# YuhuaXu/ImageMosaicing

Measured on AMD Instinct MI355X. Metric: image-pairs/sec (detect+match+H+warp), 4000x3000 UAV frames, higher is better.
Workload: dtype i16 fixed-point pyramid filtered in f32 (as the reference's OpenCV), f32 (RANSAC / warp coordinates), int8 MFMA with int32 accumulation (descriptor distances, exact), u8 (pixels); 1 GPU; C3: ONE 500-frame 4000x3000 UAV survey, pair window 2 (499 pairs), SIFT(2000,3,0.01,20) + exact BF match + 3x3 grid select + Ransac2D + MosaicImagesRefined warp; frames=500, pairs=499, frames_per_gpu=500, pairs_per_gpu=499

## Files before the change

imagemosaicing_amd/csrc/sift.hip:

```cpp
#include "common.h"
#include "sift_plan.h"
#include <memory>
#include "detmath.h"
#include <cmath>
#include <type_traits>

namespace {

using namespace sift_plan;
constexpr int MAX_INTERP = 5, ORI_BINS = 36;
constexpr int FIXPT_SCALE = 48;
constexpr float DOG_THRESHOLD_P1 = 21.0f;
constexpr float HIST_Q = 1024.0f;
constexpr int SIFT_BATCH_MAX = MI355_SIFT_BATCH_MAX;
static_assert(SIFT_BATCH_MAX == BATCH_MAX, "sift_plan.h: BATCH_MAX");
typedef int16_t lvl_t;

__host__ __device__ __forceinline__ int reflect101(int p, int n) {
    if (n == 1) return 0;
    while (p < 0 || p >= n) { if (p < 0) p = -p; else p = 2 * n - 2 - p; }
    return p;
}

typedef float v2f __attribute__((ext_vector_type(2)));
// ... 89 lines not shown
        for (int j = 1; j <= R; j++) {
            const v4f sm = *reinterpret_cast<const v4f*>(mid + j * PMID) + *reinterpret_cast<const v4f*>(mid - j * PMID);
            const v4f p = sm * a.k[R + j];
            acc = acc + p;
        }
        const int gx = x0 + 4 * xg, gy = y0 + yy;
        if (gy >= a.h) continue;
        const int o0 = sat16(acc.x), o1 = sat16(acc.y), o2 = sat16(acc.z), o3 = sat16(acc.w);
        lvl_t* d = dst + (size_t)gy * a.w + gx;
        if (gx + 3 < a.w && (a.w & 3) == 0) {
            *reinterpret_cast<uint2*>(d) = make_uint2((unsigned)(o0 & 0xffff) | ((unsigned)o1 << 16), (unsigned)(o2 & 0xffff) | ((unsigned)o3 << 16));
        } else {
            if (gx < a.w) d[0] = (lvl_t)o0;
            if (gx + 1 < a.w) d[1] = (lvl_t)o1;
            if (gx + 2 < a.w) d[2] = (lvl_t)o2;
            if (gx + 3 < a.w) d[3] = (lvl_t)o3;
        }
        if (a.ds && !(gy & 1) && (gy >> 1) < (a.h >> 1)) {
            lvl_t* q = a.ds + (size_t)fr * a.fstride + (size_t)(gy >> 1) * (a.w >> 1);
            if ((gx >> 1) < (a.w >> 1)) q[gx >> 1] = (lvl_t)o0;
            if (((gx + 2) >> 1) < (a.w >> 1)) q[(gx + 2) >> 1] = (lvl_t)o2;
        }
    }
}

#include "build/blur16_asm.inc"
template <int R, bool BGR, bool DS>
__device__ __forceinline__ void blur16_stream_body(const Blur16Args& a, int L, int nstrip, int nseg) {
    constexpr int RA = (R + 3) / 4 * 4, SW = 256, BW = SW + 2 * RA;
    constexpr int BUF = (BW + 8 + 63) & ~63;
    static_assert(2 * RA + R <= 64, "halo lanes");
    __shared__ __attribute__((aligned(16))) float s_buf[4][2][BUF];
    const int lane = threadIdx.x & 63, wave = threadIdx.x >> 6;
    int unit = __builtin_amdgcn_readfirstlane(xcd_remap(blockIdx.x, gridDim.x) * 4 + wave);
    const int per = nstrip * nseg, fr = unit / per;
    if (fr >= a.nb) return;
    unit -= fr * per;
    const int seg = unit / nstrip, strip = unit - seg * nstrip;
    if (seg >= nseg) return;
    const int x0 = strip * SW, y0 = seg * L;
    const int lact = (a.h - y0 < L) ? a.h - y0 : L;
    const int wv = a.w - x0;
    const int xm = x0 + 4 * lane;
    const int xl = xm < a.w - 4 ? xm : a.w - 4;
    int hcol, hpos;
    if (lane < RA) { hcol = x0 - RA + lane; hpos = lane; }
    else if (lane < 2 * RA) { hcol = x0 + SW + (lane - RA); hpos = SW + lane; }
    else if (wv < SW && lane < 2 * RA + R) { hcol = x0 + wv + (lane - 2 * RA); hpos = RA + wv + (lane - 2 * RA); }
    else { hcol = x0; hpos = BW + (lane & 7); }
    hcol = reflect101(hcol, a.w);
    const size_t fro = (size_t)fr * a.fstride;
    const uint8_t* bgr = a.bgr[0]; int bws = a.bgr_ws[0];
    if (BGR) {
#pragma unroll
        for (int q = 1; q < SIFT_BATCH_MAX; q++) if (fr == q) { bgr = a.bgr[q]; bws = a.bgr_ws[q]; }
    }
    const int rowb = BGR ? bws : 2 * a.w;
    int gy = y0 - R, dir = 1;
    if (gy < 0) { gy = -gy; dir = -1; }
    const unsigned long long rp = (unsigned long long)(BGR ? reinterpret_cast<uintptr_t>(bgr) : reinterpret_cast<uintptr_t>(a.src + fro)) + (unsigned long long)gy * (unsigned)rowb;
    const unsigned moff = BGR ? 3u * xl : 2u * xl;
    unsigned hoff, hsh = 0;
    if (BGR) {
        const int b0 = 3 * hcol; int st = b0 & ~3; if (st + 8 > bws) st = bws - 8;
        hoff = (unsigned)st; hsh = 8u * (unsigned)(b0 - st);
    } else hoff = 2u * hcol;
    const unsigned lds0 = (unsigned)reinterpret_cast<uintptr_t>(&s_buf[wave][0][0]);
    const unsigned lds_win = lds0 + 16u * lane, lds_main = lds0 + 4u * (RA + 4 * lane), lds_halo = lds0 + 4u * hpos;
    const unsigned long long dp = (unsigned long long)reinterpret_cast<uintptr_t>(a.dst + fro) + 2ull * (unsigned long long)y0 * a.w;
    const unsigned long long dsp = DS ? (unsigned long long)reinterpret_cast<uintptr_t>(a.ds + fro) + 2ull * (unsigned long long)(y0 >> 1) * (a.w >> 1) : 0ull;
    const unsigned doff = 2u * xm, dsoff = 2u * (xm >> 1);
    const unsigned long long smask = __ballot(xm < a.w);
    const unsigned long long kp = (unsigned long long)reinterpret_cast<uintptr_t>(__builtin_amdgcn_kernarg_segment_ptr()) + offsetof(Blur16Args, kp);
    const int n = lact + 2 * R + 1;
    const int hm1 = a.h - 1, dstr = 2 * a.w;
    (void)hsh;
#define BLUR_ASM_CALL(NAME) NAME(lds_win, lds_main, lds_halo, moff, hoff, doff, dsoff, rp, dp, dsp, kp, smask, rowb, gy, dir, hm1, dstr, n)
    if constexpr (BGR) { static_assert(R == 6, "base level"); blur16_asm_r6_bgr(lds_win, lds_main, lds_halo, moff, hoff, doff, dsoff, hsh, rp, dp, dsp, kp, smask, rowb, gy, dir, hm1, dstr, n); }
    else if constexpr (R == 5) BLUR_ASM_CALL(blur16_asm_r5);
    else if constexpr (R == 6) BLUR_ASM_CALL(blur16_asm_r6);
    else if constexpr (R == 8 && DS) BLUR_ASM_CALL(blur16_asm_r8_ds);
    else if constexpr (R == 8) BLUR_ASM_CALL(blur16_asm_r8);
    else if constexpr (R == 10) BLUR_ASM_CALL(blur16_asm_r10);
    else if constexpr (R == 13) BLUR_ASM_CALL(blur16_asm_r13);
#undef BLUR_ASM_CALL
}
template <int R, bool BGR, bool DS, int W>
__global__ __launch_bounds__(256) __attribute__((amdgpu_waves_per_eu(W, W))) void blur16_stream(Blur16Args a, int L, int nstrip, int nseg) {
    blur16_stream_body<R, BGR, DS>(a, L, nstrip, nseg);
}

__global__ __launch_bounds__(256) void downsample16(const lvl_t* src, int sw, lvl_t* dst, int dw, int dh, size_t fstride) {
    src += (size_t)blockIdx.z * fstride; dst += (size_t)blockIdx.z * fstride;
    const int x = blockIdx.x * 64 + (threadIdx.x & 63), y = blockIdx.y * 4 + (threadIdx.x >> 6);
    if (x < dw && y < dh) dst[(size_t)y * dw + x] = src[(size_t)(2 * y) * sw + 2 * x];
}

struct OctaveDev { lvl_t* lv[N_LEVELS]; int w, h; };

constexpr int ECAP = 128;
constexpr int REG_STRIDE = 32;
struct BatchStride { size_t pyr, claimed, cand, refined, kps, cube, sel, mins; };
struct FrameOuts { mi355_keypoint* kp[SIFT_BATCH_MAX]; uint8_t* d8[SIFT_BATCH_MAX]; };

struct Refined { int o, layer, r, c; float xi, xr, xc, contr, scl; unsigned start; };

struct PyrDev { OctaveDev oc[MAX_OCT]; unsigned* claimed[MAX_OCT]; unsigned* mins[MAX_OCT]; int n_oct; };

__device__ __forceinline__ float dogv(const OctaveDev& oc, size_t foff, int lvl, int r, int c) {
    const size_t o = foff + (size_t)r * oc.w + c;
    return (float)((int)oc.lv[lvl + 1][o] - (int)oc.lv[lvl][o]);
}

__device__ __forceinline__ void solve3(const float a[3][3], const float b[3], float x[3]) {
    const float det = (a[0][0] * (a[1][1] * a[2][2] - a[2][1] * a[1][2]) - a[0][1] * (a[1][0] * a[2][2] - a[2][0] * a[1][2])) + a[0][2] * (a[1][0] * a[2][1] - a[2][0] * a[1][1]);
    if (det == 0.0f) { x[0] = x[1] = x[2] = 0.0f; return; }
    const float d = 1.0f / det;
    x[0] = d * ((b[0] * (a[1][1] * a[2][2] - a[1][2] * a[2][1]) - a[0][1] * (b[1] * a[2][2] - a[1][2] * b[2])) + a[0][2] * (b[1] * a[2][1] - a[1][1] * b[2]));
    x[1] = d * ((a[0][0] * (b[1] * a[2][2] - a[1][2] * b[2]) - b[0] * (a[1][0] * a[2][2] - a[1][2] * a[2][0])) + a[0][2] * (a[1][0] * b[2] - b[1] * a[2][0]));
    x[2] = d * ((a[0][0] * (a[1][1] * b[2] - b[1] * a[2][1]) - a[0][1] * (a[1][0] * b[2] - b[1] * a[2][0])) + b[0] * (a[1][0] * a[2][1] - a[1][1] * a[2][0]));
}

struct FitOff { float xi, xr, xc; };
template <class DV>
__device__ __forceinline__ FitOff fit_step(DV dv, int L, int R, int C) {
    const float img_scale = 1.0f / (float)(255 * FIXPT_SCALE);
    const float deriv_scale = img_scale * 0.5f, second_scale = img_scale, cross_scale = img_scale * 0.25f;
    float dD[3];
    dD[0] = (dv(L, R, C + 1) - dv(L, R, C - 1)) * deriv_scale;
    dD[1] = (dv(L, R + 1, C) - dv(L, R - 1, C)) * deriv_scale;
    dD[2] = (dv(L + 1, R, C) - dv(L - 1, R, C)) * deriv_scale;
    const float v2 = dv(L, R, C) * 2.0f;
    const float dxx = (dv(L, R, C + 1) + dv(L, R, C - 1) - v2) * second_scale;
    const float dyy = (dv(L, R + 1, C) + dv(L, R - 1, C) - v2) * second_scale;
    const float dss = (dv(L + 1, R, C) + dv(L - 1, R, C) - v2) * second_scale;
    const float dxy = (dv(L, R + 1, C + 1) - dv(L, R + 1, C - 1) - dv(L, R - 1, C + 1) + dv(L, R - 1, C - 1)) * cross_scale;
    const float dxs = (dv(L + 1, R, C + 1) - dv(L + 1, R, C - 1) - dv(L - 1, R, C + 1) + dv(L - 1, R, C - 1)) * cross_scale;
    const float dys = (dv(L + 1, R + 1, C) - dv(L + 1, R - 1, C) - dv(L - 1, R + 1, C) + dv(L - 1, R - 1, C)) * cross_scale;
    const float A[3][3] = {{dxx, dxy, dxs}, {dxy, dyy, dys}, {dxs, dys, dss}};
    float X[3];
    solve3(A, dD, X);
    FitOff f; f.xi = -X[2]; f.xr = -X[1]; f.xc = -X[0];
    return f;
}
template <class DV>
__device__ __forceinline__ bool fit_accept(DV dv, int L, int R, int C, FitOff f, float contrast_thr, float edge_thr, float& contr) {
    const float img_scale = 1.0f / (float)(255 * FIXPT_SCALE);
    const float deriv_scale = img_scale * 0.5f, second_scale = img_scale, cross_scale = img_scale * 0.25f;
    float dD0 = (dv(L, R, C + 1) - dv(L, R, C - 1)) * deriv_scale;
    float dD1 = (dv(L, R + 1, C) - dv(L, R - 1, C)) * deriv_scale;
    float dD2 = (dv(L + 1, R, C) - dv(L - 1, R, C)) * deriv_scale;
    const float t = ((0.0f + dD0 * f.xc) + dD1 * f.xr) + dD2 * f.xi;
    contr = dv(L, R, C) * img_scale + t * 0.5f;
    if (fabsf(contr) * (float)N_LAYERS < contrast_thr) return false;
    const float v2 = dv(L, R, C) * 2.0f;
    const float dxx = (dv(L, R, C + 1) + dv(L, R, C - 1) - v2) * second_scale;
    const float dyy = (dv(L, R + 1, C) + dv(L, R - 1, C) - v2) * second_scale;
    const float dxy = (dv(L, R + 1, C + 1) - dv(L, R + 1, C - 1) - dv(L, R - 1, C + 1) + dv(L, R - 1, C - 1)) * cross_scale;
    const float tr = dxx + dyy, det = dxx * dyy - dxy * dxy;
    if (det <= 0.0f || (tr * tr) * edge_thr >= ((edge_thr + 1.0f) * (edge_thr + 1.0f)) * det) return false;
    return true;
}
__device__ __forceinline__ int fit_state(FitOff f) {
    if (fabsf(f.xi) < 0.5f && fabsf(f.xr) < 0.5f && fabsf(f.xc) < 0.5f) return 0;
    if (fabsf(f.xi) > 7.0e8f || fabsf(f.xr) > 7.0e8f || fabsf(f.xc) > 7.0e8f) return 1;
    if (!(f.xi == f.xi) || !(f.xr == f.xr) || !(f.xc == f.xc)) return 1;
    return 2;
}

__global__ __launch_bounds__(256) void extrema_kernel(OctaveDev oc, int octave, unsigned long long* cand, unsigned* count, unsigned cap, unsigned* overflow, BatchStride bs,
                                                      float* cube, unsigned cube_cap) {
    {
        const size_t f = blockIdx.y;
#pragma unroll
        for (int l = 0; l < N_LEVELS; l++) oc.lv[l] += f * bs.pyr;
        cand += f * bs.cand; count += f * CCNT_STRIDE; overflow += f * CNT_STRIDE; cube += f * bs.cube;
    }
    constexpr int PC = EW + 8;
    constexpr int P4 = PC / 4;
    constexpr int RW = EH + 2;
    __shared__ v4f s_d4[5][RW * P4];
    __shared__ unsigned long long s_list[ECAP];
    __shared__ unsigned s_n, s_base;
    const int tid = threadIdx.x;
    const int tiles_x = (oc.w + EW - 1) / EW, tiles_y = (oc.h + EH - 1) / EH;
    const int tile = xcd_remap(blockIdx.x, tiles_x * tiles_y);
    const int tyy = tile / tiles_x, txx = tile - tyy * tiles_x;
    const int x0 = txx * EW, y0 = tyy * EH;
    if (tid == 0) s_n = 0;
    const bool vec = ((oc.w & 3) == 0) && (x0 - 4 >= 0) && (x0 + EW + 4 <= oc.w) && ((reinterpret_cast<uintptr_t>(oc.lv[0]) & 7) == 0);
    if (vec) {
        for (int idx = tid; idx < RW * (EW / 4); idx += 256) {
            const int ry = idx / (EW / 4), c4 = idx - ry * (EW / 4);
            int gy = y0 - 1 + ry;
            gy = gy < 0 ? 0 : (gy > oc.h - 1 ? oc.h - 1 : gy);
            const size_t o = (size_t)gy * oc.w + (x0 + 4 * c4);
            v4f g[N_LEVELS];
#pragma unroll
            for (int l = 0; l < N_LEVELS; l++) g[l] = ld4(oc.lv[l] + o);
#pragma unroll
            for (int l = 0; l < 5; l++) s_d4[l][ry * P4 + 1 + c4] = g[l + 1] - g[l];
        }
        if (tid < 2 * RW) {
            const int ry = tid >> 1, side = tid & 1;
            int gy = y0 - 1 + ry;
            gy = gy < 0 ? 0 : (gy > oc.h - 1 ? oc.h - 1 : gy);
            const size_t o = (size_t)gy * oc.w + (side ? x0 + EW : x0 - 1);
            float g[N_LEVELS];
#pragma unroll
            for (int l = 0; l < N_LEVELS; l++) g[l] = ld1(oc.lv[l] + o);
#pragma unroll
            for (int l = 0; l < 5; l++) reinterpret_cast<float*>(s_d4[l])[ry * PC + (side ? 4 + EW : 3)] = g[l + 1] - g[l];
        }
    } else {
        for (int idx = tid; idx < RW * PC; idx += 256) {
            const int ry = idx / PC, rx = idx - ry * PC;
            int gy = y0 - 1 + ry, gx = x0 - 4 + rx;
            gy = gy < 0 ? 0 : (gy > oc.h - 1 ? oc.h - 1 : gy);
            gx = gx < 0 ? 0 : (gx > oc.w - 1 ? oc.w - 1 : gx);
            const size_t o = (size_t)gy * oc.w + gx;
            float g[N_LEVELS];
#pragma unroll
            for (int l = 0; l < N_LEVELS; l++) g[l] = ld1(oc.lv[l] + o);
#pragma unroll
            for (int l = 0; l < 5; l++) reinterpret_cast<float*>(s_d4[l])[idx] = g[l + 1] - g[l];
        }
    }
    __syncthreads();
    for (int item = tid; item < EH * (EW / 4); item += 256) {
        const int ly = item / (EW / 4), xg = item - ly * (EW / 4);
        const int r = y0 + ly;
        float cm[5][6], cn[5][6], mid[5][6], top[5][6], bot[5][6];
#pragma unroll
        for (int pl = 0; pl < 5; pl++) {
            const float* base = reinterpret_cast<const float*>(s_d4[pl]) + (ly + 1) * PC + 4 * xg + 4;
#pragma unroll
            for (int rr = -1; rr <= 1; rr++) {
                const float* q = base + rr * PC;
                const v4f c4 = *reinterpret_cast<const v4f*>(q);
                float v[6] = {q[-1], c4.x, c4.y, c4.z, c4.w, q[4]};
#pragma unroll
                for (int j = 0; j < 6; j++) { if (rr == -1) top[pl][j] = v[j]; else if (rr == 0) mid[pl][j] = v[j]; else bot[pl][j] = v[j]; }
            }
#pragma unroll
            for (int j = 0; j < 6; j++) {
                cm[pl][j] = fmaxf(fmaxf(top[pl][j], mid[pl][j]), bot[pl][j]);
                cn[pl][j] = fminf(fminf(top[pl][j], mid[pl][j]), bot[pl][j]);
            }
        }
        unsigned hit = 0;
#pragma unroll
        for (int k = 0; k < 4; k++) {
            const int j = k + 1;
#pragma unroll
            for (int layer = 1; layer <= N_LAYERS; layer++) {
                const float val = mid[layer][j];
                float mx = fmaxf(fmaxf(cm[layer - 1][j - 1], cm[layer - 1][j]), cm[layer - 1][j + 1]);
                mx = fmaxf(mx, fmaxf(fmaxf(cm[layer + 1][j - 1], cm[layer + 1][j]), cm[layer + 1][j + 1]));
                mx = fmaxf(mx, fmaxf(fmaxf(cm[layer][j - 1], cm[layer][j + 1]), fmaxf(top[layer][j], bot[layer][j])));
                float mn = fminf(fminf(cn[layer - 1][j - 1], cn[layer - 1][j]), cn[layer - 1][j + 1]);
                mn = fminf(mn, fminf(fminf(cn[layer + 1][j - 1], cn[layer + 1][j]), cn[layer + 1][j + 1]));
                mn = fminf(mn, fminf(fminf(cn[layer][j - 1], cn[layer][j + 1]), fminf(top[layer][j], bot[layer][j])));
                const float q = val > 0.0f ? mx : -mn;
                hit |= fabsf(val) >= fmaxf(q, DOG_THRESHOLD_P1) ? (1u << ((layer - 1) * 4 + k)) : 0u;
            }
        }
        unsigned cmask = 0;
#pragma unroll
        for (int k = 0; k < 4; k++) { const int c = x0 + 4 * xg + k; cmask |= (c >= IMG_BORDER && c < oc.w - IMG_BORDER) ? (0x111u << k) : 0u; }
        hit = (r >= IMG_BORDER && r < oc.h - IMG_BORDER) ? (hit & cmask) : 0u;
        while (hit) {
            const int bb = __builtin_ctz(hit); hit &= hit - 1;
            const int layer = bb / 4 + 1, c = x0 + 4 * xg + (bb & 3);
            const unsigned long long rec = ((unsigned long long)octave << 48) | ((unsigned long long)layer << 40) | ((unsigned long long)r << 20) | (unsigned long long)c;
            const unsigned slot = atomicAdd(&s_n, 1u);
            if (slot < ECAP) s_list[slot] = rec;
            else {
                const unsigned reg = ((unsigned)tile >> REG_SHIFT) & (NREG - 1);
                const unsigned g = atomicAdd(&count[reg * REG_STRIDE], 1u);
                if (g < cap) cand[(size_t)reg * cap + g] = rec; else *overflow = 1;
            }
        }
    }
    __syncthreads();
    const unsigned nloc = s_n < ECAP ? s_n : ECAP;
    const unsigned reg = ((unsigned)tile >> REG_SHIFT) & (NREG - 1);
    if (tid == 0 && nloc) s_base = atomicAdd(&count[reg * REG_STRIDE], nloc);
    __syncthreads();
    for (unsigned i = tid; i < nloc; i += 256) {
        const unsigned g = s_base + i;
        if (g < cap) cand[(size_t)reg * cap + g] = s_list[i] | (g < cube_cap ? (1ull << 63) : 0ull); else *overflow = 1;
    }
    for (unsigned idx = tid; idx < nloc * 27; idx += 256) {
        const unsigned ci = idx / 27, e = idx - ci * 27;
        const unsigned g = s_base + ci;
        if (g >= cube_cap) continue;
        const unsigned long long rec = s_list[ci];
        const int L0 = (int)((rec >> 40) & 0xff), R0 = (int)((rec >> 20) & 0xfffff), C0 = (int)(rec & 0xfffff);
        const int dl = (int)(e / 9) - 1, dr = (int)((e / 3) % 3) - 1, dc = (int)(e % 3) - 1;
        cube[((size_t)reg * 32 + e) * cube_cap + g] = reinterpret_cast<const float*>(s_d4[L0 + dl])[(R0 + dr - y0 + 1) * PC + (C0 + dc - x0) + 4];
    }
}

constexpr int XCAP = 512;
typedef short s2 __attribute__((ext_vector_type(2)));
struct XRow { uint2 m[N_LEVELS]; };
struct XDog { s2 m[5][2]; };
__device__ __forceinline__ s2 as_s2(unsigned v) { return __builtin_bit_cast(s2, v); }
__device__ __forceinline__ unsigned as_u(s2 v) { return __builtin_bit_cast(unsigned, v); }
__device__ __forceinline__ s2 pmax(s2 a, s2 b) { return __builtin_elementwise_max(a, b); }
__device__ __forceinline__ s2 pmin(s2 a, s2 b) { return __builtin_elementwise_min(a, b); }
__device__ __forceinline__ unsigned dpp_lower(unsigned v) { return (unsigned)__builtin_amdgcn_update_dpp(0, (int)v, 0x138 , 0xf, 0xf, true); }
__device__ __forceinline__ unsigned dpp_upper(unsigned v) { return (unsigned)__builtin_amdgcn_update_dpp(0, (int)v, 0x130 , 0xf, 0xf, true); }

__device__ __forceinline__ unsigned xtest_row(const XDog& A, const XDog& B, const XDog& C, int xm, int clo, int chi, bool row_ok) {
    s2 hx[5][2], hn[5][2];
#pragma unroll
    for (int p = 0; p < 5; p++) {
        auto h3 = [](s2 c01, s2 c23, bool mx, s2& o01, s2& o23) {
            const unsigned u01 = as_u(c01), u23 = as_u(c23);
            const unsigned l23 = dpp_lower(u23), r01 = dpp_upper(u01);
            const s2 s_m0 = as_s2(__builtin_amdgcn_alignbit(u01, l23, 16));
            const s2 s_12 = as_s2(__builtin_amdgcn_alignbit(u23, u01, 16));
            const s2 s_34 = as_s2(__builtin_amdgcn_alignbit(r01, u23, 16));
            if (mx) { o01 = pmax(pmax(s_m0, c01), s_12); o23 = pmax(pmax(s_12, c23), s_34); }
            else    { o01 = pmin(pmin(s_m0, c01), s_12); o23 = pmin(pmin(s_12, c23), s_34); }
        };
        h3(pmax(pmax(A.m[p][0], B.m[p][0]), C.m[p][0]), pmax(pmax(A.m[p][1], B.m[p][1]), C.m[p][1]), true, hx[p][0], hx[p][1]);
        h3(pmin(pmin(A.m[p][0], B.m[p][0]), C.m[p][0]), pmin(pmin(A.m[p][1], B.m[p][1]), C.m[p][1]), false, hn[p][0], hn[p][1]);
    }
    unsigned hit = 0;
    const s2 t21 = {21, 21}, tm21 = {-21, -21};
#pragma unroll
    for (int layer = 1; layer <= N_LAYERS; layer++) {
#pragma unroll
        for (int r = 0; r < 2; r++) {
            const s2 val = B.m[layer][r];
            const s2 mx = pmax(pmax(pmax(hx[layer - 1][r], hx[layer][r]), hx[layer + 1][r]), t21);
            const s2 mn = pmin(pmin(pmin(hn[layer - 1][r], hn[layer][r]), hn[layer + 1][r]), tm21);
            const bool h0 = (val.x == mx.x) | (val.x == mn.x), h1 = (val.y == mx.y) | (val.y == mn.y);
            hit = (hit << 2) | (h0 ? 2u : 0u) | (h1 ? 1u : 0u);
        }
    }
    if (!row_ok || hit == 0) return 0u;
    unsigned out = 0;
#pragma unroll
    for (int b = 0; b < 12; b++) out |= ((hit >> (11 - b)) & 1u) << b;
    unsigned cmask = 0;
#pragma unroll
    for (int k = 0; k < 4; k++) cmask |= (xm + k >= clo && xm + k < chi) ? (0x111u << k) : 0u;
    return out & cmask;
}

struct XH { s2 hx[5][2], hn[5][2]; };
struct XCen { s2 v[3][2]; };
__device__ __forceinline__ void xrow_extremes(const XDog& d, XH& h, XCen& c) {
#pragma unroll
    for (int p = 0; p < 5; p++) {
        const unsigned u01 = as_u(d.m[p][0]), u23 = as_u(d.m[p][1]);
        const unsigned l23 = dpp_lower(u23), r01 = dpp_upper(u01);
        const s2 s_m0 = as_s2(__builtin_amdgcn_alignbit(u01, l23, 16));
        const s2 s_12 = as_s2(__builtin_amdgcn_alignbit(u23, u01, 16));
        const s2 s_34 = as_s2(__builtin_amdgcn_alignbit(r01, u23, 16));
        h.hx[p][0] = pmax(pmax(s_m0, d.m[p][0]), s_12); h.hx[p][1] = pmax(pmax(s_12, d.m[p][1]), s_34);
        h.hn[p][0] = pmin(pmin(s_m0, d.m[p][0]), s_12); h.hn[p][1] = pmin(pmin(s_12, d.m[p][1]), s_34);
    }
#pragma unroll
    for (int l = 0; l < 3; l++) { c.v[l][0] = d.m[l + 1][0]; c.v[l][1] = d.m[l + 1][1]; }
}
__device__ __forceinline__ unsigned xtest_rows(const XH& A, const XH& B, const XH& C, const XCen& cen, int xm, int clo, int chi, bool row_ok) {
    s2 hx[5][2], hn[5][2];
#pragma unroll
    for (int p = 0; p < 5; p++)
#pragma unroll
        for (int r = 0; r < 2; r++) { hx[p][r] = pmax(pmax(A.hx[p][r], B.hx[p][r]), C.hx[p][r]); hn[p][r] = pmin(pmin(A.hn[p][r], B.hn[p][r]), C.hn[p][r]); }
    unsigned hit = 0;
    const s2 t21 = {21, 21}, tm21 = {-21, -21};
#pragma unroll
    for (int layer = 1; layer <= N_LAYERS; layer++) {
#pragma unroll
        for (int r = 0; r < 2; r++) {
            const s2 val = cen.v[layer - 1][r];
            const s2 mx = pmax(pmax(pmax(hx[layer - 1][r], hx[layer][r]), hx[layer + 1][r]), t21);
            const s2 mn = pmin(pmin(pmin(hn[layer - 1][r], hn[layer][r]), hn[layer + 1][r]), tm21);
            const bool h0 = (val.x == mx.x) | (val.x == mn.x), h1 = (val.y == mx.y) | (val.y == mn.y);
            hit = (hit << 2) | (h0 ? 2u : 0u) | (h1 ? 1u : 0u);
        }
    }
    if (!row_ok || hit == 0) return 0u;
    unsigned out = 0;
#pragma unroll
    for (int b = 0; b < 12; b++) out |= ((hit >> (11 - b)) & 1u) << b;
    unsigned cmask = 0;
#pragma unroll
    for (int k = 0; k < 4; k++) cmask |= (xm + k >= clo && xm + k < chi) ? (0x111u << k) : 0u;
    return out & cmask;
}

__global__ __launch_bounds__(256) __attribute__((amdgpu_waves_per_eu(XWAVES, XWAVES)))
void extrema_stream(OctaveDev oc, int octave, unsigned long long* cand, unsigned* count, unsigned cap, unsigned* overflow, BatchStride bs,
                    float* cube, unsigned cube_cap, int L, int nstrip, int nseg, int nb, int xsw ) {
    const int lane = threadIdx.x & 63, wave = threadIdx.x >> 6;
    int unit = __builtin_amdgcn_readfirstlane(xcd_remap(blockIdx.x, gridDim.x) * 4 + wave);
    const int per = nstrip * nseg, fr = unit / per;
    if (fr >= nb) return;
    unit -= fr * per;
    {
        const size_t f = (size_t)fr;
#pragma unroll
        for (int l = 0; l < N_LEVELS; l++) oc.lv[l] += f * bs.pyr;
        cand += f * bs.cand; count += f * CCNT_STRIDE; overflow += f * CNT_STRIDE; cube += f * bs.cube;
    }
    const int seg = unit / nstrip, strip = unit - seg * nstrip;
    const int xs = strip * xsw, y0 = seg * L;
    const int lact = (oc.h - y0 < L) ? oc.h - y0 : L;
    const unsigned reg = (unsigned)unit & (NREG - 1);
    const int xm = xs - 4 + 4 * lane;
    const int xl = xm < 0 ? 0 : (xm < oc.w - 4 ? xm : oc.w - 4);
    int clo = xs > IMG_BORDER ? xs : IMG_BORDER, chi = xs + xsw < oc.w - IMG_BORDER ? xs + xsw : oc.w - IMG_BORDER;
    if (lane == 0 || lane == 63) { clo = 0; chi = 0; }
    const int hm1 = oc.h - 1;
    auto load_row = [&](int r, XRow& q) {
        r = r < 0 ? 0 : (r > hm1 ? hm1 : r);
        const size_t o = (size_t)r * oc.w + xl;
#pragma unroll
        for (int l = 0; l < N_LEVELS; l++) q.m[l] = *reinterpret_cast<const uint2*>(oc.lv[l] + o);
    };
    auto to_dog = [&](const XRow& q, XDog& d) {
#pragma unroll
        for (int p = 0; p < 5; p++) { d.m[p][0] = as_s2(q.m[p + 1].x) - as_s2(q.m[p].x); d.m[p][1] = as_s2(q.m[p + 1].y) - as_s2(q.m[p].y); }
    };
    __shared__ unsigned long long s_rec[4][XCAP];
    int nq = 0;
    auto wave_sync = [&]() { __builtin_amdgcn_fence(__ATOMIC_ACQ_REL, "wavefront"); __builtin_amdgcn_wave_barrier(); };
    auto flush = [&]() {
        if (nq == 0) return;
        wave_sync();
        unsigned base = 0;
        if (lane == 0) base = atomicAdd(&count[reg * REG_STRIDE], (unsigned)nq);
        base = __shfl(base, 0);
        for (int idx = lane; idx < nq; idx += 64) {
            const unsigned g = base + (unsigned)idx;
            if (g >= cap) { *overflow = 1; continue; }
            cand[(size_t)reg * cap + g] = s_rec[wave][idx];
        }
        wave_sync();
        nq = 0;
    };
    auto emit = [&](unsigned hit, int rc, auto in_loop) -> bool {
        constexpr bool IN_LOOP = decltype(in_loop)::value;
        const int nq0 = nq;
        while (__builtin_amdgcn_ballot_w64(hit != 0)) {
            const bool mine = hit != 0;
            const int bb = mine ? __builtin_ctz(hit) : 0;
            hit &= hit - 1;
            const unsigned long long m = __builtin_amdgcn_ballot_w64(mine);
            const int add = __builtin_popcountll(m);
            if (nq + add > XCAP) {
                if constexpr (IN_LOOP) { nq = nq0; return false; }
                else flush();
            }
            if (mine) {
                const int layer = bb / 4 + 1, c = xm + (bb & 3);
                s_rec[wave][nq + __builtin_popcountll(m & ((1ull << lane) - 1ull))] =
                    ((unsigned long long)octave << 48) | ((unsigned long long)layer << 40) | ((unsigned long long)rc << 20) | (unsigned long long)c;
            }
            nq += add;
        }
        return true;
    };
    XH win[3];
    XCen cen[3];
    XRow nxt[XD];
    {
        XRow q; XDog dq;
        load_row(y0 - 1, q); to_dog(q, dq); xrow_extremes(dq, win[0], cen[0]);
        load_row(y0, q); to_dog(q, dq); xrow_extremes(dq, win[1], cen[1]);
#pragma unroll
        for (int d = 0; d < XD; d++) load_row(y0 + 1 + d, nxt[d]);
    }
    int tb = 0, t_slow = -1;
    for (bool done = false; !done;) {
        for (;;) {
            if (tb >= lact) { done = true; break; }
            if (nq > XCAP / 2) break;
            auto step = [&](auto jc) -> bool {
                constexpr int j = decltype(jc)::value;
                const int tt = tb + j;
                if (tt >= lact) return false;
                const int rc = y0 + tt;
                XH& A = win[j % 3]; XH& B = win[(j + 1) % 3]; XH& Cc = win[(j + 2) % 3];
                { XDog dq; to_dog(nxt[j % XD], dq); xrow_extremes(dq, Cc, cen[(j + 2) % 3]); }
                load_row(rc + 1 + XD, nxt[j % XD]);
                const unsigned hit = xtest_rows(A, B, Cc, cen[(j + 1) % 3], xm, clo, chi, rc >= IMG_BORDER && rc < oc.h - IMG_BORDER);
                if (!emit(hit, rc, std::true_type{})) { t_slow = tt; return false; }
                return true;
            };
            if (!static_rows<0, 3 * XD>(step)) { done = true; break; }
            tb += 3 * XD;
        }
        flush();
    }
    if (t_slow >= 0) {
        for (int tt = t_slow; tt < lact; tt++) {
            const int rc = y0 + tt;
            XRow q; XDog A, B, Cc;
            load_row(rc - 1, q); to_dog(q, A);
            load_row(rc, q); to_dog(q, B);
            load_row(rc + 1, q); to_dog(q, Cc);
            emit(xtest_row(A, B, Cc, xm, clo, chi, rc >= IMG_BORDER && rc < oc.h - IMG_BORDER), rc, std::false_type{});
        }
        flush();
    }
}

__global__ __launch_bounds__(256) void refine_kernel(PyrDev P, const unsigned long long* cand_all, const unsigned* cand_counts, unsigned cand_cap, unsigned* cand_total,
                                                     float contrast_thr, float edge_thr, float sigma,
                                                     Refined* out, unsigned* out_count, unsigned out_cap, unsigned* out_resp, BatchStride bs,
                                                     const float* cube_all, unsigned cube_cap) {
    const size_t fr = blockIdx.z, foff = fr * bs.pyr;
    cube_all += fr * bs.cube;
    cand_all += fr * bs.cand; cand_counts += fr * CCNT_STRIDE; cand_total += fr * CNT_STRIDE;
    out += fr * bs.refined; out_count += fr * CNT_STRIDE; out_resp += fr * bs.refined;
    const unsigned reg = blockIdx.y;
    unsigned n = cand_counts[reg * REG_STRIDE];
    if (n > cand_cap) n = cand_cap;
    const unsigned long long* cand = cand_all + (size_t)reg * cand_cap;
    if (blockIdx.x == 0 && blockIdx.y == 0 && threadIdx.x < 64) {
        unsigned tot = cand_counts[threadIdx.x * REG_STRIDE];
        for (int off = 32; off > 0; off >>= 1) tot += __shfl_xor(tot, off);
        if (threadIdx.x == 0) cand_total[0] = tot;
    }
    for (unsigned i = blockIdx.x * blockDim.x + threadIdx.x; i < n; i += gridDim.x * blockDim.x) {
        const unsigned long long pk = cand[i];
        const int o = (int)((pk >> 48) & 0xff);
        int L = (int)((pk >> 40) & 0xff), R = (int)((pk >> 20) & 0xfffff), C = (int)(pk & 0xfffff);
        const unsigned start = ((unsigned)L << 28) | ((unsigned)R << 14) | (unsigned)C;
        const OctaveDev& oc = P.oc[o];
        auto dv = [&](int l, int r, int c) { return dogv(oc, foff, l, r, c); };
        FitOff f = {0.0f, 0.0f, 0.0f};
        int it = 0;
        bool alive = true, accepted = false;
        float contr = 0.0f;
        const bool from_cube = (pk >> 63) != 0;
        const bool can_gather = (oc.w & 1) == 0 && (foff & 1) == 0;
        float cv[27];
        auto gather = [&](int l, int r, int c) {
            const int a0 = (c - 1) & ~1, sh = ((c - 1) & 1) * 16;
            int v[4][9];
#pragma unroll
            for (int q = 0; q < 4; q++) {
                const lvl_t* lp = oc.lv[l - 1 + q] + foff;
#pragma unroll
                for (int dr = 0; dr < 3; dr++) {
                    const uint2_a4 wv = *reinterpret_cast<const uint2_a4*>(lp + (size_t)(r - 1 + dr) * oc.w + a0);
                    const unsigned long long ww = (((unsigned long long)wv.y << 32) | wv.x) >> sh;
                    v[q][dr * 3 + 0] = (int)(short)(ww & 0xffffu); v[q][dr * 3 + 1] = (int)(short)((ww >> 16) & 0xffffu); v[q][dr * 3 + 2] = (int)(short)((ww >> 32) & 0xffffu);
                }
            }
#pragma unroll
            for (int dl = 0; dl < 3; dl++)
#pragma unroll
                for (int e = 0; e < 9; e++) cv[dl * 9 + e] = (float)(v[dl + 1][e] - v[dl][e]);
        };
        if (from_cube || can_gather) {
            for (; it < MAX_INTERP; it++) {
                if (it == 0 && from_cube) {
                    const float* cb = cube_all + (size_t)reg * 32 * cube_cap + i;
#pragma unroll
                    for (int e = 0; e < 27; e++) cv[e] = cb[(size_t)e * cube_cap];
                } else if (can_gather) gather(L, R, C);
                else break;
                const int L0 = L, R0 = R, C0 = C;
                auto dvc = [&](int l, int r, int c) { return cv[(l - L0 + 1) * 9 + (r - R0 + 1) * 3 + (c - C0 + 1)]; };
                f = fit_step(dvc, L, R, C);
                const int stt = fit_state(f);
                if (stt == 1) { alive = false; break; }
                if (stt == 0) { accepted = fit_accept(dvc, L, R, C, f, contrast_thr, edge_thr, contr); alive = accepted; break; }
                C += (int)rintf(f.xc); R += (int)rintf(f.xr); L += (int)rintf(f.xi);
                if (L < 1 || L > N_LAYERS || C < IMG_BORDER || C >= oc.w - IMG_BORDER || R < IMG_BORDER || R >= oc.h - IMG_BORDER) { alive = false; break; }
            }
            if (!alive || (can_gather && !accepted)) continue;
        }
        if (!accepted) {
            for (; it < MAX_INTERP; it++) {
                f = fit_step(dv, L, R, C);
                const int stt = fit_state(f);
                if (stt == 0) break;
                if (stt == 1) { alive = false; break; }
                C += (int)rintf(f.xc); R += (int)rintf(f.xr); L += (int)rintf(f.xi);
                if (L < 1 || L > N_LAYERS || C < IMG_BORDER || C >= oc.w - IMG_BORDER || R < IMG_BORDER || R >= oc.h - IMG_BORDER) { alive = false; break; }
            }
            if (!alive || it >= MAX_INTERP) continue;
            if (!fit_accept(dv, L, R, C, f, contrast_thr, edge_thr, contr)) continue;
        }
        const size_t bit = ((size_t)R * oc.w + C) * 4 + (size_t)L;
        const unsigned mask = 1u << (bit & 31);
        if (!P.mins[o]) {
            const unsigned old = atomicOr(&P.claimed[o][fr * bs.claimed + (bit >> 5)], mask);
            if (old & mask) continue;
        }
        const unsigned long long act = __ballot(1);
        const int leader = __builtin_ctzll(act), lane_id = (int)(threadIdx.x & 63);
        unsigned slot = 0;
        if (lane_id == leader) slot = atomicAdd(out_count, (unsigned)__builtin_popcountll(act));
        slot = __shfl(slot, leader) + (unsigned)__builtin_popcountll(act & ((1ull << lane_id) - 1ull));
        if (slot < out_cap) {
            Refined rr;
            rr.o = o; rr.layer = L; rr.r = R; rr.c = C; rr.xi = f.xi; rr.xr = f.xr; rr.xc = f.xc; rr.contr = contr;
            rr.scl = sigma * det_exp2f(((float)L + f.xi) / (float)N_LAYERS);
            rr.start = start;
            out[slot] = rr;
            out_resp[slot] = __float_as_uint(fabsf(contr));
            if (P.mins[o]) atomicMin(&P.mins[o][fr * bs.mins + bit], start);
        } else if (!P.mins[o]) atomicAnd(&P.claimed[o][fr * bs.claimed + (bit >> 5)], ~mask);
    }
}

__device__ __forceinline__ void unclaim_body(const PyrDev& P, const Refined* ref, const unsigned* ref_count, unsigned ref_cap, const BatchStride& bs, size_t fr, unsigned first, unsigned step) {
    ref += fr * bs.refined; ref_count += fr * CNT_STRIDE;
    unsigned n = *ref_count;
    if (n > ref_cap) n = ref_cap;
    for (unsigned i = first; i < n; i += step) {
        const Refined rr = ref[i];
        const size_t bit = ((size_t)rr.r * P.oc[rr.o].w + rr.c) * 4 + (size_t)rr.layer;
        atomicAnd(&P.claimed[rr.o][fr * bs.claimed + (bit >> 5)], ~(1u << (bit & 31)));
    }
}

__global__ __launch_bounds__(256) void keepall_live_kernel(PyrDev P, const Refined* ref, const unsigned* ref_count, unsigned ref_cap, unsigned* ctrl, unsigned* list, BatchStride bs) {
    const size_t fr = blockIdx.y;
    ref += fr * bs.refined; ref_count += fr * CNT_STRIDE; ctrl += fr * CNT_STRIDE; list += fr * bs.refined;
    unsigned n = *ref_count;
    if (n > ref_cap) n = ref_cap;
    const int lane = threadIdx.x & 63;
    for (unsigned i0 = blockIdx.x * blockDim.x; i0 < n; i0 += gridDim.x * blockDim.x) {
        const unsigned i = i0 + threadIdx.x;
        bool take = false;
        if (i < n) {
            const Refined rr = ref[i];
            const size_t bit = ((size_t)rr.r * P.oc[rr.o].w + rr.c) * 4 + (size_t)rr.layer;
            take = P.mins[rr.o][fr * bs.mins + bit] == rr.start;
        }
        const unsigned long long m = __builtin_amdgcn_ballot_w64(take);
        if (m) {
            const int first = __builtin_ctzll(m);
            unsigned base = 0;
            if (lane == first) base = atomicAdd(&ctrl[2], (unsigned)__builtin_popcountll(m));
            base = __shfl(base, first);
            if (take) list[base + (unsigned)__builtin_popcountll(m & ((1ull << lane) - 1ull))] = i;
        }
    }
}
__global__ __launch_bounds__(256) void keepall_reset_kernel(PyrDev P, const Refined* ref, const unsigned* ref_count, unsigned ref_cap, BatchStride bs) {
    const size_t fr = blockIdx.y;
    ref += fr * bs.refined; ref_count += fr * CNT_STRIDE;
    unsigned n = *ref_count;
    if (n > ref_cap) n = ref_cap;
    for (unsigned i = blockIdx.x * blockDim.x + threadIdx.x; i < n; i += gridDim.x * blockDim.x) {
        const Refined rr = ref[i];
        P.mins[rr.o][fr * bs.mins + ((size_t)rr.r * P.oc[rr.o].w + rr.c) * 4 + (size_t)rr.layer] = 0xffffffffu;
    }
}

struct KpRec {
    unsigned resp_bits; int o, layer, r, c, bin;
    float ptx, pty, scl, angle, xi;
    unsigned start;
};

constexpr int UNCLAIM_WGS = 32;
__global__ __launch_bounds__(1024) void select_unclaim_kernel(PyrDev P, const Refined* ref, BatchStride bs,
                                                              const unsigned* resp , const unsigned* ref_count, unsigned ref_cap,
                                                              unsigned want, unsigned* ctrl , size_t resp_stride,
                                                              unsigned* list ) {
    if (blockIdx.x > 0) { unclaim_body(P, ref, ref_count, ref_cap, bs, blockIdx.y, (blockIdx.x - 1) * 1024 + threadIdx.x, (gridDim.x - 1) * 1024); return; }
    resp += (size_t)blockIdx.y * resp_stride; ref_count += (size_t)blockIdx.y * CNT_STRIDE; ctrl += (size_t)blockIdx.y * CNT_STRIDE;
    list += (size_t)blockIdx.y * resp_stride;
    __shared__ unsigned s_h[16][256];
    __shared__ unsigned s_sel[2], s_cnt;
    const int tid = threadIdx.x, wv = tid >> 6;
    unsigned n = *ref_count;
    if (n > ref_cap) n = ref_cap;
    if (n <= want) {
        if (tid == 0) { ctrl[0] = 0; ctrl[1] = 0; ctrl[2] = n; }
        for (unsigned i = tid; i < n; i += 1024) list[i] = i;
        return;
    }
    const unsigned nr = (n + 1023u) & ~1023u;
    unsigned above = 0, hi_sel = 0;
    for (int pass = 0; pass < 2; pass++) {
        for (int i = tid; i < 16 * 256; i += 1024) (&s_h[0][0])[i] = 0;
        __syncthreads();
        for (unsigned i0 = tid; i0 < nr; i0 += 8 * 1024) {
            unsigned vv[8];
#pragma unroll
            for (int u = 0; u < 8; u++) { const unsigned i = i0 + 1024u * u; vv[u] = i < n ? resp[i] : 0u; }
#pragma unroll
            for (int u = 0; u < 8; u++) {
                if (i0 + 1024u * u >= n) continue;
                const unsigned key = (vv[u] >> 15) & 0xffffu;
                if (pass == 0) atomicAdd(&s_h[wv][key >> 8], 1u);
                else if ((key >> 8) == hi_sel) atomicAdd(&s_h[wv][key & 255u], 1u);
            }
        }
        __syncthreads();
        if (tid < 256) { unsigned t = 0; for (int w = 0; w < 16; w++) t += s_h[w][tid]; s_h[0][tid] = t; }
        __syncthreads();
        if (tid == 0) {
            unsigned cum = above; int b = 255;
            for (; b >= 0; b--) { if (cum + s_h[0][b] >= want) break; cum += s_h[0][b]; }
            if (b < 0) b = 0;
            s_sel[0] = (unsigned)b; s_sel[1] = cum;
        }
        __syncthreads();
        if (pass == 0) { hi_sel = s_sel[0]; above = s_sel[1]; }
        else if (tid == 0) { ctrl[0] = ((hi_sel << 8) | s_sel[0]) << 15; ctrl[1] = 0; s_cnt = 0; }
        __syncthreads();
    }
    const unsigned T = ((hi_sel << 8) | s_sel[0]) << 15;
    const int lane = tid & 63;
    for (unsigned i0 = tid; i0 < nr; i0 += 8 * 1024) {
        unsigned vv[8];
#pragma unroll
        for (int u = 0; u < 8; u++) { const unsigned i = i0 + 1024u * u; vv[u] = i < n ? resp[i] : 0u; }
#pragma unroll
        for (int u = 0; u < 8; u++) {
            const unsigned i = i0 + 1024u * u;
            const bool take = i < n && vv[u] >= T;
            const unsigned long long m = __builtin_amdgcn_ballot_w64(take);
            if (m) {
                const int first = __builtin_ctzll(m);
                unsigned base = 0;
                if (lane == first) base = atomicAdd(&s_cnt, (unsigned)__builtin_popcountll(m));
                base = __shfl(base, first);
                if (take) list[base + (unsigned)__builtin_popcountll(m & ((1ull << lane) - 1ull))] = i;
            }
        }
    }
    __syncthreads();
    if (tid == 0) ctrl[2] = s_cnt;
}

constexpr int OCAP = 256;
__global__ __launch_bounds__(256) void orient_kernel(PyrDev P, const Refined* ref, const unsigned* ref_count, unsigned ref_cap,
                                                     KpRec* out, unsigned* out_resp, unsigned* out_count, unsigned out_cap,
                                                     const unsigned* ctrl, int pass, BatchStride bs, const unsigned* list) {
    const size_t fr = blockIdx.y, foff = fr * bs.pyr;
    ref += fr * bs.refined; ref_count += fr * CNT_STRIDE; out += fr * bs.kps; out_resp += fr * bs.kps; out_count += fr * CNT_STRIDE; ctrl += fr * CNT_STRIDE;
    list += fr * bs.refined;
    __shared__ unsigned long long s_hq[4][ORI_BINS];
    const unsigned Tbits = ctrl[0];
    if (pass == 1 && (ctrl[1] == 0 || Tbits == 0)) return;
    __shared__ float s_hist[4][ORI_BINS + 4];
    __shared__ KpRec s_out[OCAP];
    __shared__ unsigned s_on, s_obase;
    const int tid = threadIdx.x, lane = tid & 63, wv = tid >> 6;
    unsigned n = *ref_count;
    if (n > ref_cap) n = ref_cap;
    if (pass == 0) n = ctrl[2] < n ? ctrl[2] : n;
    if (tid == 0) s_on = 0;
    __syncthreads();
    for (unsigned base = blockIdx.x * 4; base < n; base += gridDim.x * 4) {
        unsigned k = base + wv;
        bool take = false;
        if (k < n) {
            if (pass == 0) { k = list[k]; take = true; }
            else take = __float_as_uint(fabsf(ref[k].contr)) < Tbits;
        }
        if (take) {
            const Refined rr = ref[k];
            const OctaveDev& oc = P.oc[rr.o];
            const lvl_t* img = oc.lv[rr.layer] + foff;
            const int radius = (int)rintf(4.5f * rr.scl);
            const float osig = 1.5f * rr.scl;
            const float expf_scale = -1.0f / (2.0f * osig * osig);
            const int side = 2 * radius + 1, S = side * side;
            if (lane < ORI_BINS) s_hq[wv][lane] = 0ull;
            __builtin_amdgcn_fence(__ATOMIC_ACQ_REL, "workgroup");
            __builtin_amdgcn_wave_barrier();
            const int per = (S + 63) / 64;
            int sc = lane * per, ic = sc / side, jc = sc - ic * side;
            for (int k0 = 0; k0 < per; k0 += 4) {
                float dxv[4], dyv[4]; int d2v[4]; bool okv[4];
#pragma unroll
                for (int u = 0; u < 4; u++) {
                    const int s = k0 + u < per ? sc : S;
                    const int i = ic - radius, j = jc - radius;
                    sc++; jc++;
                    if (jc == side) { jc = 0; ic++; }
                    const int y = rr.r + i, x = rr.c + j;
                    okv[u] = (s < S) && !(y <= 0 || y >= oc.h - 1 || x <= 0 || x >= oc.w - 1);
                    d2v[u] = i * i + j * j;
                    dxv[u] = 0.0f; dyv[u] = 0.0f;
                    if (okv[u]) {
                        dxv[u] = (float)((int)img[(size_t)y * oc.w + x + 1] - (int)img[(size_t)y * oc.w + x - 1]);
                        dyv[u] = (float)((int)img[(size_t)(y - 1) * oc.w + x] - (int)img[(size_t)(y + 1) * oc.w + x]);
                    }
                }
#pragma unroll
                for (int u = 0; u < 4; u++) {
                    if (!okv[u]) continue;
                    const float dx = dxv[u], dy = dyv[u];
                    const float wgt = det_expf((float)d2v[u] * expf_scale);
                    const float ang = det_atan2deg(dy, dx);
                    const float mag = sqrtf(dx * dx + dy * dy);
                    int b = (int)rintf(((float)ORI_BINS / 360.0f) * ang);
                    if (b >= ORI_BINS) b -= ORI_BINS;
                    if (b < 0) b += ORI_BINS;
                    const float t = wgt * mag;
                    atomicAdd(&s_hq[wv][b], (unsigned long long)(long long)(int)rintf(t * HIST_Q));
                }
            }
            __builtin_amdgcn_fence(__ATOMIC_ACQ_REL, "workgroup");
            __builtin_amdgcn_wave_barrier();
// ... 779 lines not shown
```

Before: 3899 image-pairs/s.

## Capture 3x3x3 DoG neighbourhood cubes in extrema stream via LDS ring

The streaming extrema kernel now keeps the last three DoG rows in a per-wave LDS ring buffer. When a candidate is emitted, it copies the 27-value neighbourhood into LDS, and the flush writes those values into the cube array, setting the cube-valid bit on each candidate. This lets refinement reuse the cubes instead of re-reading the pyramid. It also shrinks XCAP and the flush threshold so LDS stays within budget. The cost is extra LDS writes on every row, added wave syncs in emit, more frequent flushes, and cubes only for the first 64 candidates per flush.

```diff
diff --git a/imagemosaicing_amd/csrc/sift.hip b/imagemosaicing_amd/csrc/sift.hip
--- a/imagemosaicing_amd/csrc/sift.hip
+++ b/imagemosaicing_amd/csrc/sift.hip
@@ -415,7 +415,12 @@
     }
 }
 
-constexpr int XCAP = 512;
+constexpr int XCAP = 144;
+constexpr int XNB_CAP = 64;
+constexpr int XRING_DW = 5 * 3 * 128;
+constexpr int XNB_DW = 18;
+constexpr int XLDS_BYTES = 4 * (XRING_DW * 4 + XCAP * 8 + XNB_CAP * XNB_DW * 4);
+static_assert(XWAVES * XLDS_BYTES <= 160 * 1024 && XLDS_BYTES <= 53 * 1024, "extrema_stream: ring + list must leave room for XWAVES workgroups per CU");
 typedef short s2 __attribute__((ext_vector_type(2)));
 struct XRow { uint2 m[N_LEVELS]; };
 struct XDog { s2 m[5][2]; };
@@ -543,10 +548,19 @@
 #pragma unroll
         for (int p = 0; p < 5; p++) { d.m[p][0] = as_s2(q.m[p + 1].x) - as_s2(q.m[p].x); d.m[p][1] = as_s2(q.m[p + 1].y) - as_s2(q.m[p].y); }
     };
+    __shared__ unsigned s_ring[4][XRING_DW];
     __shared__ unsigned long long s_rec[4][XCAP];
+    __shared__ uint2 s_nb[4][XNB_CAP][XNB_DW / 2];
+    static_assert(sizeof(s_ring) + sizeof(s_rec) + sizeof(s_nb) == XLDS_BYTES, "XLDS_BYTES");
+    auto ring_put = [&](const XDog& d, int slot) {
+        unsigned* q = &s_ring[wave][lane * 30 + slot];
+#pragma unroll
+        for (int p = 0; p < 5; p++) { q[p * 3] = as_u(d.m[p][0]); q[p * 3 + 15] = as_u(d.m[p][1]); }
+    };
     int nq = 0;
     auto wave_sync = [&]() { __builtin_amdgcn_fence(__ATOMIC_ACQ_REL, "wavefront"); __builtin_amdgcn_wave_barrier(); };
-    auto flush = [&]() {
+    auto flush = [&](auto cubes) {
+        constexpr bool CUBES = decltype(cubes)::value;
         if (nq == 0) return;
         wave_sync();
         unsigned base = 0;
@@ -555,13 +569,28 @@
         for (int idx = lane; idx < nq; idx += 64) {
             const unsigned g = base + (unsigned)idx;
             if (g >= cap) { *overflow = 1; continue; }
-            cand[(size_t)reg * cap + g] = s_rec[wave][idx];
+            const unsigned long long rec = s_rec[wave][idx];
+            const bool has = CUBES && idx < XNB_CAP && g < cube_cap;
+            cand[(size_t)reg * cap + g] = rec | (has ? (1ull << 63) : 0ull);
+            if (has) {
+                const int sh = (rec & 1ull) ? 0 : 16;
+                float* cb = cube + (size_t)reg * 32 * cube_cap + g;
+#pragma nounroll
+                for (int i = 0; i < XNB_DW / 2; i++, cb += (size_t)3 * cube_cap) {
+                    const uint2 wv = s_nb[wave][idx][i];
+                    const unsigned long long ww = (((unsigned long long)wv.y << 32) | wv.x) >> sh;
+                    cb[0] = (float)(int)(short)(ww & 0xffffu);
+                    cb[cube_cap] = (float)(int)(short)((ww >> 16) & 0xffffu);
+                    cb[(size_t)2 * cube_cap] = (float)(int)(short)((ww >> 32) & 0xffffu);
+                }
+            }
         }
         wave_sync();
         nq = 0;
     };
-    auto emit = [&](unsigned hit, int rc, auto in_loop) -> bool {
-        constexpr bool IN_LOOP = decltype(in_loop)::value;
+    auto emit = [&](unsigned hit, int rc, auto sbc) -> bool {
+        constexpr int SB = decltype(sbc)::value;
+        constexpr bool IN_LOOP = SB >= 0;
         const int nq0 = nq;
         while (__builtin_amdgcn_ballot_w64(hit != 0)) {
             const bool mine = hit != 0;
@@ -571,12 +600,27 @@
             const int add = __builtin_popcountll(m);
             if (nq + add > XCAP) {
                 if constexpr (IN_LOOP) { nq = nq0; return false; }
-                else flush();
-            }
+                else flush(std::false_type{});
+            }
+            if constexpr (IN_LOOP) wave_sync();
             if (mine) {
-                const int layer = bb / 4 + 1, c = xm + (bb & 3);
-                s_rec[wave][nq + __builtin_popcountll(m & ((1ull << lane) - 1ull))] =
-                    ((unsigned long long)octave << 48) | ((unsigned long long)layer << 40) | ((unsigned long long)rc << 20) | (unsigned long long)c;
+                const int layer = bb / 4 + 1, k = bb & 3, c = xm + k;
+                const int slot = nq + __builtin_popcountll(m & ((1ull << lane) - 1ull));
+                s_rec[wave][slot] = ((unsigned long long)octave << 48) | ((unsigned long long)layer << 40) | ((unsigned long long)rc << 20) | (unsigned long long)c;
+                if (IN_LOOP && slot < XNB_CAP) {
+                    const unsigned* q = &s_ring[wave][(2 * lane + ((k + 1) >> 1) - 1) * 15 + (layer - 1) * 3];
+                    uint2* nbp = s_nb[wave][slot];
+                    uint2 v[XNB_DW / 2];
+#pragma unroll
+                    for (int pl = 0; pl < 3; pl++)
+#pragma unroll
+                        for (int dr = 0; dr < 3; dr++) {
+                            const int o = pl * 3 + (SB + dr + 2) % 3;
+                            v[pl * 3 + dr] = make_uint2(q[o], q[o + 15]);
+                        }
+#pragma unroll
+                    for (int i = 0; i < XNB_DW / 2; i++) nbp[i] = v[i];
+                }
             }
             nq += add;
         }
@@ -585,34 +629,35 @@
     XH win[3];
     XCen cen[3];
     XRow nxt[XD];
-    {
+    auto prime = [&](int t) {
         XRow q; XDog dq;
-        load_row(y0 - 1, q); to_dog(q, dq); xrow_extremes(dq, win[0], cen[0]);
-        load_row(y0, q); to_dog(q, dq); xrow_extremes(dq, win[1], cen[1]);
-#pragma unroll
-        for (int d = 0; d < XD; d++) load_row(y0 + 1 + d, nxt[d]);
-    }
+        load_row(y0 + t - 1, q); to_dog(q, dq); ring_put(dq, 0); xrow_extremes(dq, win[0], cen[0]);
+        load_row(y0 + t, q); to_dog(q, dq); ring_put(dq, 1); xrow_extremes(dq, win[1], cen[1]);
+#pragma unroll
+        for (int d = 0; d < XD; d++) load_row(y0 + t + 1 + d, nxt[d]);
+    };
+    prime(0);
     int tb = 0, t_slow = -1;
     for (bool done = false; !done;) {
         for (;;) {
             if (tb >= lact) { done = true; break; }
-            if (nq > XCAP / 2) break;
+            if (nq > XNB_CAP / 2) break;
             auto step = [&](auto jc) -> bool {
                 constexpr int j = decltype(jc)::value;
                 const int tt = tb + j;
                 if (tt >= lact) return false;
                 const int rc = y0 + tt;
                 XH& A = win[j % 3]; XH& B = win[(j + 1) % 3]; XH& Cc = win[(j + 2) % 3];
-                { XDog dq; to_dog(nxt[j % XD], dq); xrow_extremes(dq, Cc, cen[(j + 2) % 3]); }
+                { XDog dq; to_dog(nxt[j % XD], dq); ring_put(dq, (j + 2) % 3); xrow_extremes(dq, Cc, cen[(j + 2) % 3]); }
                 load_row(rc + 1 + XD, nxt[j % XD]);
                 const unsigned hit = xtest_rows(A, B, Cc, cen[(j + 1) % 3], xm, clo, chi, rc >= IMG_BORDER && rc < oc.h - IMG_BORDER);
-                if (!emit(hit, rc, std::true_type{})) { t_slow = tt; return false; }
+                if (!emit(hit, rc, std::integral_constant<int, (j + 1) % 3>{})) { t_slow = tt; return false; }
                 return true;
             };
             if (!static_rows<0, 3 * XD>(step)) { done = true; break; }
             tb += 3 * XD;
         }
-        flush();
+        flush(std::true_type{});
     }
     if (t_slow >= 0) {
         for (int tt = t_slow; tt < lact; tt++) {
@@ -621,9 +666,9 @@
             load_row(rc - 1, q); to_dog(q, A);
             load_row(rc, q); to_dog(q, B);
             load_row(rc + 1, q); to_dog(q, Cc);
-            emit(xtest_row(A, B, Cc, xm, clo, chi, rc >= IMG_BORDER && rc < oc.h - IMG_BORDER), rc, std::false_type{});
-        }
-        flush();
+            emit(xtest_row(A, B, Cc, xm, clo, chi, rc >= IMG_BORDER && rc < oc.h - IMG_BORDER), rc, std::integral_constant<int, -1>{});
+        }
+        flush(std::false_type{});
     }
 }
 
```

Result: faster. 4023 image-pairs/s (median of 6 runs) (+3.2%).
